# ChuaCheowHuan/gym-continuousDoubleAuction

Hardware: AMD Instinct MI355X
Metric: agent-steps/sec (whole node), 4 agents x N parallel markets; step() with every info tensor (row a14), 4 free-running group chain(s) (higher is better)
Workload: dtype int32+dec28+f64

## Files before the change

gym_continuousdoubleauction_amd/csrc/cda_book.inc:

```
constexpr int CAP = CDA_CAP;
__host__ __device__ constexpr int book_phys(int s, int i) { return s == 0 ? i : CAP - 1 - i; }
struct BookField {
    int32_t v[CAP];
    struct Row { int32_t* base; int s; __device__ __forceinline__ int32_t& operator[](int i) const { return base[book_phys(s, i)]; } };
    struct CRow { const int32_t* base; int s; __device__ __forceinline__ const int32_t& operator[](int i) const { return base[book_phys(s, i)]; } };
    __device__ __forceinline__ Row operator[](int s) { return Row{v, s}; }
    __device__ __forceinline__ CRow operator[](int s) const { return CRow{v, s}; }
};
struct Book {
    BookField price, qty;
    BookField oo;
    BookField ts;
};
constexpr int BOOK_BYTES = sizeof(Book);
enum { TL_N = 0, TL_BASE = 2, TL_PTR_LO = 4, TL_PTR_HI = 5, TL_CAP = 6, TL_ORD = 8, TL_WORDS = 12 };
struct Lds {
    Book book;
    int32_t lvl_px[2][CDA_K_ROWS];
    int32_t lvl_sz[2][CDA_K_ROWS];
    int32_t act_tsp[CDA_MAX_AGENTS];
    int32_t act_size[CDA_MAX_AGENTS];
    int32_t tl[TL_WORDS];
    Acc acc[CDA_MAX_AGENTS];
};
// ... 340 lines not shown
            if (i < tn) { T.field(s, 0)[to] = v0; T.field(s, 1)[to] = v1; T.field(s, 2)[to] = v2; T.field(s, 3)[to] = v3; }
        }
    }
    L.tl[TL_BASE + s] = base; L.tl[TL_N + s] = tn - 1;
    CDA_WSYNC();
    tail_fence();
}
CDA_COLD void cold_aggregate(uint32_t lds_addr, int s, int t, int carry) {
    Lds& L = lds_at(lds_addr);
    const Tail T = tail_of(L);
    const int lane = lane_id();
    const int base = L.tl[TL_BASE + s], tn = L.tl[TL_N + s];
    int32_t prev = t > 0 ? L.book.price[s][t - 1] : -1;
    for (int b = 0; b < tn && carry <= CDA_K_ROWS; b += WAVE) {
        const int i = b + lane;
        const bool valid = i < tn;
        int32_t p = 0, q = 0;
        if (valid) { const uint32_t sl = T.slot(base, i); p = T.field(s, 0)[sl]; q = T.field(s, 1)[sl]; }
        const int32_t up = __shfl(p, (lane + 63) & 63, WAVE);
        const int32_t pp = lane == 0 ? prev : up;
        const bool head = valid && p != pp;
        const uint64_t mk = __ballot(head);
        const uint64_t le = lane == 63 ? ~0ull : ((1ull << (lane + 1)) - 1ull);
        const int lvl = carry + __popcll(mk & le) - 1;
        if (valid && lvl >= 0 && lvl < CDA_K_ROWS) {
            atomicAdd(&L.lvl_sz[s][lvl], q);
            if (head) L.lvl_px[s][lvl] = p;
        }
        carry += __popcll(mk);
        prev = __builtin_amdgcn_readlane(p, 63);
    }
    CDA_WSYNC();
}
__device__ __forceinline__ void sync_tail_status(const Lds& L, Mkt& m) {
    m.status = (m.status & ~ST_TAIL_ANY) | (L.tl[TL_N] > 0 ? ST_TAIL_BID : 0) | (L.tl[TL_N + 1] > 0 ? ST_TAIL_ASK : 0);
}
__device__ __forceinline__ void set_counts(Mkt& m, uint32_t counts) { m.nb = (int32_t)(counts & 0x7fffu); m.na = (int32_t)((counts >> 16) & 0x7fffu); }
__device__ __forceinline__ int total_orders(const Lds& L, const Mkt& m) { return m.nb + m.na + ((m.status & ST_TAIL_ANY) ? L.tl[TL_N] + L.tl[TL_N + 1] : 0); }
#define ACC_UPD(field, expr) do { D _r = (expr); st_dec(a.field, _r, flags); } while (0)
__device__ __forceinline__ void xfer_inc(Acc& a, bool counter, D v, uint32_t& flags) {
    cda_dec& fld = counter ? a.hold : a.cash;
    D r = d_sub(ld_dec(fld), v);
    st_dec(fld, r, flags);
}
__device__ __forceinline__ void xfer_dec(Acc& a, bool counter, D v, uint32_t& flags) {
    ACC_UPD(cash, d_add(ld_dec(a.cash), v));
    if (counter) { ACC_UPD(hold, d_sub(ld_dec(a.hold), v)); ACC_UPD(cash, d_add(ld_dec(a.cash), v)); }
}
__device__ __forceinline__ D posval_from(Acc& a, uint32_t n, int32_t price, bool is_long) {
    D raw = d_mul_int(ld_dec(a.vwap), n), mkt = d_price_times(price, n);
    return d_add(raw, cal_profit(is_long, mkt, raw));
}
template <bool LAZY_POSVAL>
__device__ __forceinline__ void settle_fill(Lds& L, int tr, int counter, int32_t q, int32_t price, int init_side, uint32_t& flags, int lane CDA_TF_PARAM) {
    uint32_t f = 0;
    TF_BEGIN();
    const int al = lane_acc(lane), g = lane_grp(lane);
    if (counter != tr) {
        if ((al == tr || al == counter) && g < 3) {
            Acc& a = L.acc[al];
            const bool is_counter = al == counter;
            const int own_side = is_counter ? init_side ^ 1 : init_side;
            int4 cnt = *reinterpret_cast<const int4*>(&a.net_position);
            const D vwap0 = ld_dec(a.vwap);
            const int32_t pos = cnt.x;
            const uint32_t ap = (uint32_t)(pos < 0 ? -pos : pos);
            const bool is_long = pos > 0;
            int mode;
            if (pos == 0) mode = 0;
            else if (is_long == (own_side == S_BID)) mode = 1;
            else mode = ap > (uint32_t)q ? 2 : (ap == (uint32_t)q ? 3 : 4);
            const D tv = d_price_times(price, (uint32_t)q);
            D X = d_zero(), mkt = d_zero();
            TF_END(14);
            if (g == 0 && mode != 0) X = d_mul_int(vwap0, ap);
            TF_END(15);
            D x2 = d_zero(), y2 = d_zero();
            cda_dec* dst = nullptr;
            bool s2 = false;
            if (g == 0) {
                s2 = true;
                if (mode == 0) { x2 = ld_dec(a.posval); y2 = tv; dst = &a.posval; }
                else if (mode <= 2) { x2 = X; y2 = tv; y2.sign = mode == 2 ? 1 : 0; }
                else { mkt = d_price_times(price, ap); x2 = is_long ? mkt : X; y2 = d_neg(is_long ? X : mkt); }
            } else if (mode <= 2) {
                if (g == 1) {
                    s2 = true;
                    dst = (mode != 2 && is_counter) ? &a.hold : &a.cash;
                    x2 = ld_dec(*dst); y2 = tv; y2.sign = mode != 2 ? 1 : 0;
                } else if (mode == 2 && is_counter) {
                    s2 = true;
                    dst = &a.hold; x2 = ld_dec(a.hold); y2 = d_neg(tv);
                }
            }
            D Y = d_zero();
            TF_END(16);
            if (s2) { Y = d_add(x2, y2); if (dst) st_dec(*dst, Y, f); }
            TF_END(17);
            if (g == 0) {
                cnt.y += 1; cnt.z += 1; cnt.w += is_counter ? 1 : 0;
                if (mode == 0) st_dec(a.vwap, d_price(price), f);
                else if (mode <= 2) {
                    const uint32_t n = mode == 1 ? ap + (uint32_t)q : ap - (uint32_t)q;
                    ACC_UPD(vwap, d_div_u32(Y, n));
                    if (!LAZY_POSVAL) ACC_UPD(posval, posval_from(a, n, price, is_long));
                    if (mode == 2 && is_counter) ACC_UPD(cash, d_add(ld_dec(a.cash), tv));
                } else {
                    D pv = d_add(X, Y);
                    ACC_UPD(cash, d_add(ld_dec(a.cash), d_sub(pv, mkt)));
                    st_dec(a.posval, d_zero(), f); st_dec(a.vwap, d_zero(), f);
                    if (mode == 3) xfer_dec(a, is_counter, tv, f);
                    else {
                        xfer_dec(a, is_counter, mkt, f);
                        D npv = d_price_times(price, (uint32_t)q - ap);
                        st_dec(a.posval, npv, f); st_dec(a.vwap, d_price(price), f);
                        xfer_inc(a, is_counter, npv, f);
                    }
                }
                int64_t np = (int64_t)pos + (own_side == S_BID ? (int64_t)q : -(int64_t)q);
                if (np > 2147483647LL || np < -2147483647LL) f |= CDA_FLAG_INT_OVERFLOW << 8;
                cnt.x = (int32_t)np;
                *reinterpret_cast<int4*>(&a.net_position) = cnt;
            }
            if (mode >= 3) { TF_END(22); TF_COUNT(21); } else if (g == 0 && mode == 0) { TF_END(23); TF_COUNT(12); } else TF_END(18);
            TF_COUNT(20);
        }
        CDA_WSYNC();
        TF_WAVE(tr, counter);
        TF_RESYNC();
    } else if (lane == tr) {
        Acc& a = L.acc[lane];
        D tv = d_price_times(price, (uint32_t)q);
        D hold = d_sub(ld_dec(a.hold), tv), cash = d_add(ld_dec(a.cash), tv);
        st_dec(a.hold, hold, f); st_dec(a.cash, cash, f);
    }
    if (__ballot((f & 0xffu) != 0)) flags |= CDA_FLAG_DEC_DOMAIN;
    if (__ballot((f >> 8) != 0)) flags |= CDA_FLAG_INT_OVERFLOW;
    TF_END(19);
    TF_WAVE_END();
}

template <bool TAILS, bool LAZY_POSVAL>
__device__ __forceinline__ int32_t match(Lds& L, Mkt& m, int tr, int own_side, int32_t qty, int32_t limit, int lane) {
    int opp = own_side ^ 1;
    Book& bk = L.book;
    for (;;) {
        int h = 0;
        const int nopp = mkt_n(m, opp);
        while (qty > 0 && h < nopp) {
            int32_t p = bk.price[opp][h];
            if (limit >= 0) { if (own_side == S_BID ? !(limit >= p) : !(limit <= p)) break; }
            int32_t rq = bk.qty[opp][h], c = oo_owner(bk.oo[opp][h]), f;
            if (qty < rq) { f = qty; bk.qty[opp][h] = rq - qty; qty = 0; CDA_WSYNC(); }
            else { f = rq; qty -= rq; h++; }
            m.has_trade = 1; m.last_trade_price = p;
            TACC_COUNT(m, 5, 1);
            m.fills += 1;
            if (m.fills == 1) __builtin_amdgcn_s_setprio(1);
            else if (m.fills == 2) __builtin_amdgcn_s_setprio(2);
            else if (m.fills == 3) __builtin_amdgcn_s_setprio(3);
            if (!CDA_MKT_DBG(m, 0x1000)) settle_fill<LAZY_POSVAL>(L, tr, c, f, p, own_side, m.flags, lane CDA_TF_ARG(m));
        }
        if (h) { book_remove(bk, opp, nopp, 0, h, lane); mkt_set_n(m, opp, nopp - h); }
        if constexpr (TAILS) {
            if (!mkt_has_tail(m, opp)) break;
            const bool ran_out = qty > 0 && h == nopp;
            set_counts(m, cold_rebalance(lds_addr_of(L), pack_counts(m.nb, m.na)));
            sync_tail_status(L, m);
            if (!ran_out || mkt_n(m, opp) == 0) break;
        } else break;
    }
    return qty;
}

__device__ __forceinline__ void cash_hold_transfer(Lds& L, int tr, int32_t price, int32_t qty, int cash_dir, uint32_t& flags, int lane) {
    const int g = lane_grp(lane);
    if (lane_acc(lane) == tr && g < 2) {
        Acc& a = L.acc[tr];
        D v = d_price_times(price, (uint32_t)qty);
        cda_dec& fld = g == 0 ? a.cash : a.hold;
        v.sign = (g == 0) == (cash_dir > 0) ? 0 : 1;
        const D cur = ld_dec(fld);
        D r = d_add_order_value(cur, v);
        if (r.exp == D_NOT_HANDLED) r = d_add(cur, v);
        st_dec(fld, r, flags);
    }
    CDA_WSYNC();
}

__device__ __forceinline__ bool order_approved(Lds& L, const Mkt& m, int tr, int side, int32_t size, int32_t price, int lane) {
    int ok = 0;
    if (lane == tr) {
        const Acc& a = L.acc[lane];
        const D nav = ld_dec(a.nav), cash = ld_dec(a.cash);
        const int32_t pos32 = a.net_position;
        const int32_t opp_best = L.book.price[side ^ 1][0];
        if (d_sgn(nav) > 0) {
            int64_t pos = pos32, opening;
            int64_t apos = pos < 0 ? -pos : pos;
            if ((side == S_BID && pos >= 0) || (side == S_ASK && pos <= 0)) opening = size;
            else { opening = (int64_t)size - apos; if (opening < 0) opening = 0; }
            if (opening <= 0) ok = 1;
            else {
                D est;
                if (price < 0) {
                    int opp = side ^ 1;
                    if (mkt_n(m, opp) > 0) est = d_price(opp_best);
                    else if (m.has_trade) est = d_price(m.last_trade_price);
                    else est = d_from_u32(1);
                } else est = d_price(price);
                uint64_t ov = (uint64_t)((uint32_t)est.w0) * (uint64_t)opening;
                int kdig = est.exp - cash.exp;
                int bc = bits128(d_c128(cash)), bo = 64 - __clzll(ov | 1ull);
                if (!cash.sign && kdig >= 0 && kdig <= 30 && opening < (1LL << 31) && bc - 1 >= bo + ((kdig * 3402) >> 10) + 1) ok = 1;
                else ok = d_cmp(cash, d_mul_u32(est, (uint32_t)opening, 0)) >= 0;
            }
        }
    }
    return __ballot(ok != 0) != 0;
}

template <bool TAILS, bool LAZY_POSVAL>
__device__ __forceinline__ void place_order(Lds& L, Mkt& m, int tr, int type, int side, int32_t size, int32_t price, int lane) {
    if (side == S_NONE) return;
// ... 189 lines not shown
```

gym_continuousdoubleauction_amd/csrc/cda_dec.hpp:

```cpp
#pragma once
#include <hip/hip_runtime.h>
#include <stdint.h>

typedef unsigned __int128 u128;

namespace cda {

#ifdef CDA_DEC_COUNTERS
__device__ unsigned long long g_dec_calls[8];
#define DEC_COUNT(i) atomicAdd(&g_dec_calls[i], 1ull)
#else
#define DEC_COUNT(i) do {} while (0)
#endif

template <int NL> struct WN { uint32_t w[NL]; };
typedef WN<8> W;
typedef WN<4> W4;

struct D {
    uint32_t w0, w1, w2;
    int32_t exp;
    int32_t sign;
};

// ... 187 lines not shown
__device__ __forceinline__ D d_from_i64(int64_t v) {
    uint64_t a = v < 0 ? (uint64_t)(-(v + 1)) + 1u : (uint64_t)v;
    return d_make((uint32_t)a, (uint32_t)(a >> 32), 0, 0, v < 0);
}
__device__ __forceinline__ D d_from_u32(uint32_t v) { return d_make(v, 0, 0, 0, 0); }
__device__ __forceinline__ D d_price(int32_t p) { uint64_t a = (uint64_t)(uint32_t)p * 10u; return d_make((uint32_t)a, (uint32_t)(a >> 32), 0, -1, 0); }
__device__ __forceinline__ D d_price_times(int32_t p, uint32_t n) {
    const uint64_t c = (uint64_t)(uint32_t)p * 10u * (uint64_t)n;
    return d_make((uint32_t)c, (uint32_t)(c >> 32), 0, -1, 0);
}
__device__ __forceinline__ bool d_is_zero(const D& a) { return (a.w0 | a.w1 | a.w2) == 0; }
template <int NL> __device__ __forceinline__ WN<NL> d_wide(const D& a) { return w_from3<NL>(a.w0, a.w1, a.w2); }
__device__ __forceinline__ D d_neg(D a) { a.sign ^= 1; return a; }
__device__ __forceinline__ int d_sgn(const D& a) { return d_is_zero(a) ? 0 : (a.sign ? -1 : 1); }

template <int NL> __device__ __forceinline__ D d_fix_impl(int sign, WN<NL> x, int exp) {
    if (w_is_zero(x)) return d_make(0, 0, 0, exp, sign);
    int nd = w_ndigits(x);
    if (nd > 28) {
        int drop = nd - 28;
        bool sticky = false;
        int k = drop;
        while (k > 9) { sticky |= (w_divc<1000000000u>(x) != 0); k -= 9; }
        uint32_t rem = w_div_pow10_small(x, k);
        uint32_t half = 5u * pow10_sel(k - 1);
        bool up = rem > half || (rem == half && (sticky || (x.w[0] & 1u)));
        if (up) {
            w_inc(x);
            if (x.w[0] == 0x10000000u && x.w[1] == 0x3e250261u && x.w[2] == 0x204fce5eu) {
                x.w[0] = 0xe8000000u; x.w[1] = 0x9fd0803cu; x.w[2] = 0x033b2e3cu; drop += 1;
            }
        }
        exp += drop;
    }
    return d_make(x.w[0], x.w[1], x.w[2], exp, sign);
}
__device__ __noinline__ D d_fix_mid(int sign, W4 x, int exp) { DEC_COUNT(0); return d_fix_impl<4>(sign, x, exp); }
__device__ __noinline__ D d_fix_wide(int sign, W x, int exp) { DEC_COUNT(1); return d_fix_impl<8>(sign, x, exp); }

__device__ __forceinline__ u128 d_c128(const D& a) { return ((u128)a.w2 << 64) | ((u128)a.w1 << 32) | (u128)a.w0; }
__device__ __forceinline__ D d_from128(u128 c, int exp, int sign) { return d_make((uint32_t)c, (uint32_t)(c >> 32), (uint32_t)(c >> 64), exp, sign); }
__device__ __forceinline__ W4 w4_from128(u128 c) { W4 r; r.w[0] = (uint32_t)c; r.w[1] = (uint32_t)(c >> 32); r.w[2] = (uint32_t)(c >> 64); r.w[3] = (uint32_t)(c >> 96); return r; }
__device__ __forceinline__ u128 p28_128() { return ((u128)0x204fce5eULL << 64) | 0x3e25026110000000ULL; }
__device__ __forceinline__ int bits128(u128 c) {
    uint64_t hi = (uint64_t)(c >> 64), lo = (uint64_t)c;
    return hi ? 128 - __clzll(hi) : (lo ? 64 - __clzll(lo) : 0);
}
__device__ __forceinline__ u128 mul_pow10_128(u128 x, int k) {
    while (k >= 9) { x *= (u128)1000000000u; k -= 9; }
    return x * (u128)pow10_sel(k);
}
__device__ __forceinline__ bool scale_fits128(u128 c, int k) { return bits128(c) + ((k * 3402) >> 10) + 1 <= 126; }

__device__ __noinline__ D d_round_mid(int sign, u128 r, int exp) {
    DEC_COUNT(2);
    const int t = (bits128(r) * 1233) >> 12;
    const int d0 = t - 28, d0c = d0 > 9 ? 9 : d0, d1c = d0 + 1 > 9 ? 9 : d0 + 1;
    const lds_u32p pt = lds_pow10(t);
    const uint32_t t0 = pt[0], t1 = pt[1], t2 = pt[2], t3 = pt[3];
    const uint32_t pw_a = lds_pow10(d0c)[0], pw_b = lds_pow10(d1c)[0];
    const double rd_a = lds_rcp10(d0c), rd_b = lds_rcp10(d1c);
    const u128 pw_t = ((u128)t3 << 96) | ((u128)t2 << 64) | ((u128)t1 << 32) | (u128)t0;
    const bool more = r >= pw_t;
    int drop = d0 + (more ? 1 : 0);
    exp += drop;
    W4 x = w4_from128(r);
    bool sticky = false;
    uint32_t pw = more ? pw_b : pw_a;
    double rd = more ? rd_b : rd_a;
    if (drop > 9) {
        const int pre = drop - 9;
        sticky = w_div_small(x, lds_pow10(pre)[0], lds_rcp10(pre)) != 0;
        drop = 9; pw = 1000000000u; rd = lds_rcp10(9);
    }
    WN<3> q; q.w[0] = x.w[0]; q.w[1] = x.w[1]; q.w[2] = x.w[2];
    const uint32_t rem = w_div_small_seeded(q, pw, rd, x.w[3]);
    const uint32_t half = pw >> 1;
    const bool up = rem > half || (rem == half && (sticky || (q.w[0] & 1u) != 0));
    const uint64_t s0 = (uint64_t)q.w[0] + (up ? 1u : 0u);
    const uint64_t s1 = (uint64_t)q.w[1] + (s0 >> 32);
    uint32_t w0 = (uint32_t)s0, w1 = (uint32_t)s1, w2 = q.w[2] + (uint32_t)(s1 >> 32);
    const bool ten28 = w0 == 0x10000000u && w1 == 0x3e250261u && w2 == 0x204fce5eu;
    w0 = ten28 ? 0xe8000000u : w0; w1 = ten28 ? 0x9fd0803cu : w1; w2 = ten28 ? 0x033b2e3cu : w2;
    exp += ten28 ? 1 : 0;
    return d_make(w0, w1, w2, exp, sign);
}

__device__ __noinline__ D d_add_wide(D a, D b) {
    DEC_COUNT(3);
    int exp = a.exp < b.exp ? a.exp : b.exp;
    bool az = d_is_zero(a), bz = d_is_zero(b);
    if (az && bz) return d_make(0, 0, 0, exp, a.sign < b.sign ? a.sign : b.sign);
    if (az || bz) {
        D o = az ? b : a;
        int e = exp > o.exp - 29 ? exp : o.exp - 29;
        W x = d_wide<8>(o);
        w_mul_pow10(x, o.exp - e);
        return d_fix_wide(o.sign, x, e);
    }
    bool swp = a.exp < b.exp;
    D dt = swp ? b : a, dO = swp ? a : b;
    W xt = d_wide<8>(dt), xo = d_wide<8>(dO);
    int et = dt.exp, eo = dO.exp;
    if (et != eo) {
        int tmp_len = w_ndigits(xt), oth_len = w_ndigits(xo);
        int m = tmp_len - 30; if (m > -1) m = -1;
        int e = et + m;
        if (oth_len + eo - 1 < e) { xo = w_from3<8>(1, 0, 0); eo = e; }
        w_mul_pow10(xt, et - eo);
    }
    W r; int rs;
    if (dt.sign != dO.sign) {
        int c = w_cmp(xt, xo);
        if (c == 0) return d_make(0, 0, 0, exp, 0);
        if (c > 0) { r = w_sub(xt, xo); rs = dt.sign; } else { r = w_sub(xo, xt); rs = dO.sign; }
    } else { r = w_add(xt, xo); rs = dt.sign; }
    return d_fix_wide(rs, r, eo);
}
__device__ __noinline__ D d_add_mid(D a, D b) {
    DEC_COUNT(4);
    bool swp = a.exp < b.exp;
    D t = swp ? b : a, o = swp ? a : b;
    int diff = t.exp - o.exp;
    u128 ct = d_c128(t), co = d_c128(o);
    bool ok = true;
    if (diff) {
        int lb_adj = o.exp + (((bits128(co) - 1) * 1233) >> 12);
        ok = scale_fits128(ct, diff) && lb_adj >= t.exp - 1;
    }
    if (!ok) return d_add_wide(a, b);
    if (diff) ct = mul_pow10_128(ct, diff);
    u128 r; int rs;
    if (t.sign != o.sign) {
        if (ct == co) return d_make(0, 0, 0, o.exp, 0);
        if (ct > co) { r = ct - co; rs = t.sign; } else { r = co - ct; rs = o.sign; }
    } else { r = ct + co; rs = t.sign; }
    if (r < p28_128()) return d_from128(r, o.exp, rs);
    return d_round_mid(rs, r, o.exp);
}
__device__ __forceinline__ u128 mul_u32_pow10_lds(uint32_t c, int k) {
    const lds_u32p p = lds_pow10(k);
    u128 pw = ((u128)p[2] << 64) | ((u128)p[1] << 32) | (u128)p[0];
    return pw * (u128)c;
}
__device__ __forceinline__ D d_add(D a, D b) {
    const bool az = d_is_zero(a), bz = d_is_zero(b);
    if (!az && !bz) {
        const bool swp = a.exp < b.exp;
        const D t = swp ? b : a, o = swp ? a : b;
        const int diff = t.exp - o.exp;
        const u128 co = d_c128(o);
        u128 ct;
        bool ok;
        if (diff == 0) { ct = d_c128(t); ok = true; }
        else {
            ok = (((bits128(co) - 1) * 1233) >> 12) >= diff - 1;
            if ((t.w1 | t.w2) == 0 && diff <= 28) ct = mul_u32_pow10_lds(t.w0, diff);
            else if (diff <= 9) ct = d_c128(t) * (u128)lds_pow10(diff)[0];
            else { ok = false; ct = 0; }
        }
        if (ok) {
            u128 r; int rs;
            if (t.sign != o.sign) {
                if (ct == co) return d_make(0, 0, 0, o.exp, 0);
                if (ct > co) { r = ct - co; rs = t.sign; } else { r = co - ct; rs = o.sign; }
            } else { r = ct + co; rs = t.sign; }
            if (r < p28_128()) return d_from128(r, o.exp, rs);
            return d_round_mid(rs, r, o.exp);
        }
        return d_add_mid(a, b);
    }
    if (az != bz) {
        const D o = az ? b : a, z = az ? a : b;
        if (z.exp >= o.exp) return o;
    }
    return d_add_wide(a, b);
}
__device__ __forceinline__ D d_sub(D a, D b) { return d_add(a, d_neg(b)); }
constexpr int D_NOT_HANDLED = -0x40000000;
__device__ __noinline__ D d_add_order_value(D field, D v) {
    const int diff = v.exp - field.exp;
    const u128 co = d_c128(field);
    const bool fz = co == 0;
    const int dcl = diff < 0 ? 0 : (diff > 28 ? 28 : diff);
    const bool shape = (v.w1 | v.w2) == 0 && v.w0 != 0 && diff == dcl &&
                       (fz || (((bits128(co) - 1) * 1233) >> 12) >= diff - 1);
    const u128 ct = mul_u32_pow10_lds(v.w0, dcl);
    const bool same = field.sign == v.sign || fz;
    const bool vg = ct > co;
    const u128 sum = ct + co, dv = ct - co, df = co - ct;
    const u128 r = same ? sum : (vg ? dv : df);
    int rs = same ? (fz ? v.sign : field.sign) : (vg ? v.sign : field.sign);
    rs = r == 0 ? 0 : rs;
    const bool ok = shape && r < p28_128();
    return d_make(ok ? (uint32_t)r : 0u, ok ? (uint32_t)(r >> 32) : 0u, ok ? (uint32_t)(r >> 64) : 0u, ok ? field.exp : D_NOT_HANDLED, ok ? rs : 0);
}

__device__ __forceinline__ D d_mul_u32(D a, uint32_t m, int mexp) {
    int exp = a.exp + mexp;
    if (d_is_zero(a) || m == 0) return d_make(0, 0, 0, exp, a.sign);
    u128 p = d_c128(a) * (u128)m;
    if (p < p28_128()) return d_from128(p, exp, a.sign);
    return d_round_mid(a.sign, p, exp);
}
__device__ __forceinline__ D d_mul_int(D a, uint32_t n) { return d_mul_u32(a, n, 0); }

template <int NL> __device__ __forceinline__ uint32_t w_mod5(const WN<NL>& x) {
    uint64_t sacc = 0;
    #pragma unroll
    for (int i = 0; i < NL; i++) sacc += x.w[i];
    return (uint32_t)(sacc % 5u);
}
template <int NL> __device__ __forceinline__ D d_div_impl(D a, uint32_t n, int shift) {
    WN<NL> x = d_wide<NL>(a);
    int exp = a.exp - shift;
    w_mul_pow10(x, shift);
    uint32_t rem = w_div_u32(x, n);
    if (rem != 0) {
        if (w_mod5(x) == 0) w_inc(x);
        WN<NL> p29 = w_pow10<NL>(29);
        const bool d30 = w_cmp(x, p29) >= 0;
        uint32_t dg, half;
        if (d30) { dg = w_divc<100u>(x); half = 50u; exp += 2; } else { dg = w_divc<10u>(x); half = 5u; exp += 1; }
        if (dg > half || (dg == half && (x.w[0] & 1u))) {
            w_inc(x);
            if (x.w[0] == 0x10000000u && x.w[1] == 0x3e250261u && x.w[2] == 0x204fce5eu) {
                x.w[0] = 0xe8000000u; x.w[1] = 0x9fd0803cu; x.w[2] = 0x033b2e3cu; exp += 1;
            }
        }
        return d_make(x.w[0], x.w[1], x.w[2], exp, a.sign);
    }
    int ideal = a.exp;
    while (exp + 9 <= ideal) { WN<NL> t = x; if (w_divc<1000000000u>(t) != 0) break; x = t; exp += 9; }
    while (exp < ideal) { WN<NL> t = x; if (w_divc<10u>(t) != 0) break; x = t; exp += 1; }
    return d_fix_impl<NL>(a.sign, x, exp);
}
__device__ __noinline__ D d_div_general(D a, uint32_t n) {
    DEC_COUNT(5);
    if (d_is_zero(a)) return d_make(0, 0, 0, a.exp, a.sign);
    {
        WN<3> x; x.w[0] = a.w0; x.w[1] = a.w1; x.w[2] = a.w2;
        if (w_div_u32(x, n) == 0) return d_make(x.w[0], x.w[1], x.w[2], a.exp, a.sign);
    }
    W4 xa = d_wide<4>(a), xn = w_from3<4>(n, 0, 0);
    int ln = w_ndigits(xn);
    int shift = ln - w_ndigits(xa) + 29;
    if (ln <= 9) return d_div_impl<4>(a, n, shift);
    return d_div_impl<8>(a, n, shift);
}
__device__ __forceinline__ int ndigits_u32(uint32_t n) {
    int d = 1;
    d = n >= 10u ? 2 : d; d = n >= 100u ? 3 : d; d = n >= 1000u ? 4 : d; d = n >= 10000u ? 5 : d; d = n >= 100000u ? 6 : d;
    d = n >= 1000000u ? 7 : d; d = n >= 10000000u ? 8 : d; d = n >= 100000000u ? 9 : d; d = n >= 1000000000u ? 10 : d;
    return d;
}
__device__ __noinline__ D d_div_pos_leaf(D a, uint32_t n) {
    DEC_COUNT(6);
    if (n - 1u >= (1u << 30) - 1u) return d_make(0, 0, 0, D_NOT_HANDLED, 0);
    const double rn = 1.0 / (double)n;
    const u128 c = d_c128(a);
    WN<3> q; q.w[0] = a.w0; q.w[1] = a.w1; q.w[2] = a.w2;
    int s = 0;
    if (w_div_small(q, n, rn) != 0) {
        const int t = (bits128(c) * 1233) >> 12;
        const lds_u32p pt = lds_pow10(t);
        const u128 pw_t = ((u128)pt[2] << 64) | ((u128)pt[1] << 32) | (u128)pt[0];
        const int s0 = 27 + ndigits_u32(n) - (t + (c >= pw_t ? 1 : 0));
        const lds_u32p ps = lds_pow10(s0);
        const u128 pw_s = ((u128)ps[3] << 96) | ((u128)ps[2] << 64) | ((u128)ps[1] << 32) | (u128)ps[0];
        const u128 x0 = c * pw_s;
        const u128 n27 = (u128)n * (((u128)0x033b2e3cULL << 64) | 0x9fd0803ce8000000ULL);
        const bool d28 = x0 >= n27;
        s = s0 + (d28 ? 0 : 1);
        W4 x = w4_from128(d28 ? x0 : x0 * 10u);
        const uint32_t r = w_div_small(x, n, rn);
        q.w[0] = x.w[0]; q.w[1] = x.w[1]; q.w[2] = x.w[2];
        if (r != 0) {
            const uint32_t twice = r * 2u;
            const bool up = twice > n || (twice == n && (q.w[0] & 1u) != 0);
            const uint64_t s0w = (uint64_t)q.w[0] + (up ? 1u : 0u);
            const uint64_t s1w = (uint64_t)q.w[1] + (s0w >> 32);
            uint32_t w0 = (uint32_t)s0w, w1 = (uint32_t)s1w, w2 = q.w[2] + (uint32_t)(s1w >> 32);
            const bool ten28 = w0 == 0x10000000u && w1 == 0x3e250261u && w2 == 0x204fce5eu;
            w0 = ten28 ? 0xe8000000u : w0; w1 = ten28 ? 0x9fd0803cu : w1; w2 = ten28 ? 0x033b2e3cu : w2;
            return d_make(w0, w1, w2, a.exp - s + (ten28 ? 1 : 0), a.sign);
        }
        #pragma unroll 1
        while (s >= 4) { WN<3> u = q; if (w_divc<10000u>(u) != 0) break; q = u; s -= 4; }
        #pragma unroll 1
        while (s >= 1) { WN<3> u = q; if (w_divc<10u>(u) != 0) break; q = u; s -= 1; }
    }
    return d_make(q.w[0], q.w[1], q.w[2], a.exp - s, a.sign);
}
__device__ __forceinline__ D d_div_u32(D a, uint32_t n) {
    D r = d_div_pos_leaf(a, n);
    if (r.exp == D_NOT_HANDLED) r = d_div_general(a, n);
    return r;
}

__device__ __noinline__ int d_cmp_wide(D a, D b) {
    int s = a.sign ? -1 : 1;
    int diff = a.exp - b.exp;
    if (diff >= 28) return s;
    if (diff <= -28) return -s;
    W xa = d_wide<8>(a), xb = d_wide<8>(b);
    if (diff > 0) w_mul_pow10(xa, diff); else if (diff < 0) w_mul_pow10(xb, -diff);
    int c = w_cmp(xa, xb);
    return c == 0 ? 0 : (c > 0 ? s : -s);
}
__device__ __noinline__ int d_cmp_mid(D a, D b) {
    int s = a.sign ? -1 : 1;
    int diff = a.exp - b.exp;
    u128 ca = d_c128(a), cb = d_c128(b);
    if (diff > 0) { if (!scale_fits128(ca, diff)) return d_cmp_wide(a, b); ca = mul_pow10_128(ca, diff); }
    else if (diff < 0) { if (!scale_fits128(cb, -diff)) return d_cmp_wide(a, b); cb = mul_pow10_128(cb, -diff); }
    return ca == cb ? 0 : (ca > cb ? s : -s);
}
__device__ __forceinline__ int d_cmp(D a, D b) {
    const bool az = d_is_zero(a), bz = d_is_zero(b);
    if (az) return bz ? 0 : (b.sign ? 1 : -1);
    if (bz) return a.sign ? -1 : 1;
    if (a.sign != b.sign) return a.sign ? -1 : 1;
    const int s = a.sign ? -1 : 1;
    const bool swp = a.exp < b.exp;
    const D t = swp ? b : a, o = swp ? a : b;
    const int diff = t.exp - o.exp;
    const bool short_t = (t.w1 | t.w2) == 0;
    if (!(short_t ? diff <= 28 : diff <= 9)) return d_cmp_mid(a, b);
    const lds_u32p p = lds_pow10(diff);
    const uint32_t p0 = p[0], p1 = p[1], p2 = p[2];
    const u128 big = short_t ? (((u128)p2 << 64) | ((u128)p1 << 32) | (u128)p0) : d_c128(t);
    const u128 ct = big * (u128)(short_t ? t.w0 : p0), co = d_c128(o);
    const int c = ct == co ? 0 : (ct > co ? s : -s);
    return swp ? -c : c;
}

__device__ __forceinline__ double round_quotient(uint64_t q, bool sticky, int t, int k) {
    int nb = 64 - __clzll(q);
    int sh = nb - 53;
    uint64_t mant = q >> sh;
    uint64_t low = q & (((uint64_t)1 << sh) - 1);
    uint64_t half = (uint64_t)1 << (sh - 1);
    if (low > half || (low == half && (sticky || (mant & 1)))) mant += 1;
    return ldexp((double)mant, t - 56 + sh - k);
}
__device__ __forceinline__ void w_shl(W& x, int n) {
    int ws = n >> 5, bs = n & 31;
    W r;
// ... 142 lines not shown
```

gym_continuousdoubleauction_amd/csrc/cda_hip.hip:

```cpp
#include <hip/hip_runtime.h>
#include <stdint.h>
#include <stdio.h>
#include <stdlib.h>
#include <string.h>
#include <math.h>
#include <dlfcn.h>

#include "../../include/cda.h"
#include "../../include/cda_random_agents.h"
#include "cda_dec.hpp"
#include "cda_market.hpp"
#include <type_traits>
#include <mutex>
#include "../../include/cda_mlp.h"
namespace cda { namespace mlpdev {
#include "cda_mlp_dev.inc"
} }
#undef CDA_MLP_HIST
#define CDA_MLP_HIST 1
namespace cda { namespace mlpdev_h1 {
#include "cda_mlp_dev.inc"
} }
#undef CDA_MLP_HIST
#define CDA_MLP_HIST 2
// ... 424 lines not shown
        cda_random_action(seed, market_base + (uint64_t)mk, (uint32_t)(step0 + (int)t), (uint32_t)a, &category[ix], &size_mean[ix], &size_sigma[ix], &price[ix], &price_offset[ix]);
    }
}
__global__ __launch_bounds__(256) void k_handback_unpack(const uint8_t* rec, int n_seg, int seg_records, long long seg_row_stride, long long row0, int A, int H, int stride,
                                                          long long n_rows_total, float* obs_full, double* reward_full, uint8_t* term_full, uint8_t* trunc_full) {
    const long long r = (long long)(((size_t)blockIdx.x * blockDim.x + threadIdx.x) >> 6);
    const int lane = (int)(threadIdx.x & 63);
    if (r >= (long long)n_seg * seg_records) return;
    const uint8_t* p = rec + (size_t)r * (size_t)stride;
    const long long seg = r / seg_records, local = row0 + (r % seg_records);
    if (n_rows_total > 0 && local >= (seg == n_seg - 1 ? n_rows_total - seg * seg_row_stride : seg_row_stride)) return;
    const size_t row = (size_t)(seg * seg_row_stride + local);
    const uint8_t* fl = p + CDA_SNAPSHOT_DIM * 4 + A * 8;
    const bool restarted = fl[2] != 0;
    if (lane < CDA_SNAPSHOT_DIM) {
        float* o = obs_full + row * (size_t)(H * CDA_SNAPSHOT_DIM);
        const float nf = reinterpret_cast<const float*>(p)[lane];
        float keep[CDA_MAX_HIST];
        #pragma unroll
        for (int h = 1; h < CDA_MAX_HIST; h++) keep[h] = h < H ? o[h * CDA_SNAPSHOT_DIM + lane] : 0.0f;
        #pragma unroll
        for (int h = 1; h < CDA_MAX_HIST; h++) if (h < H) o[(h - 1) * CDA_SNAPSHOT_DIM + lane] = restarted ? nf : keep[h];
        o[(H - 1) * CDA_SNAPSHOT_DIM + lane] = nf;
    }
    if (lane < A) reward_full[row * (size_t)A + (size_t)lane] = reinterpret_cast<const double*>(p + CDA_SNAPSHOT_DIM * 4)[lane];
    if (lane == 0) { term_full[row] = fl[0]; trunc_full[row] = fl[1]; }
}
__global__ void k_book_peak(const uint8_t* arena, Params P, int32_t* out) {
    int i = (int)(blockIdx.x * blockDim.x + threadIdx.x);
    if (i < P.n_markets) out[i] = (int32_t)((const uint32_t*)(arena + (size_t)i * (size_t)P.lay.stride))[H_PEAK_ORDERS];
}

__global__ void k_selftest_dec(int op, int n, const cda_dec* a, const cda_dec* b, cda_dec* out) {
    int i = (int)(blockIdx.x * blockDim.x + threadIdx.x);
    dec_tables_init();
    if (i >= n) return;
    D x = ld_dec(a[i]);
    D y = b ? ld_dec(b[i]) : d_zero();
    cda_dec o; o.w[0] = o.w[1] = o.w[2] = 0; o.exp = 0; o.sign = 0; o.pad = 0;
    uint32_t f = 0;
    uint32_t yc = y.w0;
    switch (op) {
        case 0: st_dec(o, d_add(x, y), f); break;
        case 1: st_dec(o, d_sub(x, y), f); break;
        case 2: { D r = d_mul_u32(x, yc, y.exp); r.sign ^= y.sign; st_dec(o, r, f); break; }
        case 3: { D r = d_div_u32(x, yc); r.sign ^= y.sign; st_dec(o, r, f); break; }
        case 4: o.w[0] = (uint32_t)(d_cmp(x, y) + 1); break;
        case 6: {
            D r = d_add_order_value(x, y);
            const bool handled = r.exp != D_NOT_HANDLED;
            if (!handled) r = d_add(x, y);
            st_dec(o, r, f); o.pad = handled ? 1u : 0u; break;
        }
        default: { double d = d_to_double(x, &f); unsigned long long bits = (unsigned long long)__double_as_longlong(d); o.w[0] = (uint32_t)bits; o.w[1] = (uint32_t)(bits >> 32); o.w[2] = f; break; }
    }
    out[i] = o;
}
__global__ void k_selftest_libm(int op, int n, const double* x, double* y) {
    int i = (int)(blockIdx.x * blockDim.x + threadIdx.x);
    if (i < n) y[i] = op == 0 ? glibc_log1p(x[i]) : (op == 1 ? glibc_exp(x[i]) : sqrt(x[i]));
}
__global__ void k_selftest_rng(uint64_t seed, int lo, int hi, int n_steps, int n_normals, int perm_n,
                               int32_t* first_int, double* normals, int32_t* perms, uint64_t* final_state) {
    if (threadIdx.x != 0 || blockIdx.x != 0) return;
    Mkt m; rng_seed(m, seed);
    *first_int = rng_integers(m, lo, hi);
    for (int s = 0; s < n_steps; s++) {
        for (int k = 0; k < n_normals; k++) normals[(size_t)s * (size_t)n_normals + (size_t)k] = rng_std_normal(m);
        int32_t* p = perms + (size_t)s * (size_t)perm_n;
        for (int i = 0; i < perm_n; i++) p[i] = i;
        for (int i = perm_n - 1; i >= 1; i--) { int j = (int)rng_interval(m, (uint32_t)i); int32_t t = p[i]; p[i] = p[j]; p[j] = t; }
    }
    final_state[0] = (uint64_t)(m.rng_state >> 64); final_state[1] = (uint64_t)m.rng_state;
    final_state[2] = (uint64_t)(m.rng_inc >> 64); final_state[3] = (uint64_t)m.rng_inc;
    final_state[4] = m.has_u32; final_state[5] = m.uinteger;
}

struct cda_env {
    Params P;
    int device;
    int cap;
    uint8_t* arena;
    size_t arena_bytes;
    uint8_t* done_buf;
    uint8_t* handback;
    int64_t hb_row_stride, hb_rows_total;
    int32_t spill_wanted;
    double* em_partials;
    MktRow* rows;
    cda_market_params* rows_host;
    uint32_t* snap_flag;
};
static inline int32_t handback_stride_of(int32_t num_agents) { return (CDA_SNAPSHOT_DIM * 4 + num_agents * 8 + 3 + 7) & ~7; }

static thread_local char g_err[256] = "";
static int g_dbg_skip = 0;
static unsigned long long* g_phase_cycles = NULL;
static int hip_fail(hipError_t e, const char* what) {
    snprintf(g_err, sizeof g_err, "%s: %s", what, hipGetErrorString(e));
    return CDA_ERR_HIP;
}
#define HIPCHK(x) do { hipError_t _e = (x); if (_e != hipSuccess) return hip_fail(_e, #x); } while (0)

extern "C" {

const char* cda_strerror(int status) {
// ... 745 lines not shown
        }
        h[H_PEAK_ORDERS] = (uint32_t)(s->n_bids + s->n_asks);
    }
    h[H_RNG_STATE_LO] = (uint32_t)s->rng_state_lo; h[H_RNG_STATE_LO + 1] = (uint32_t)(s->rng_state_lo >> 32);
    h[H_RNG_STATE_HI] = (uint32_t)s->rng_state_hi; h[H_RNG_STATE_HI + 1] = (uint32_t)(s->rng_state_hi >> 32);
    h[H_RNG_INC_LO] = (uint32_t)s->rng_inc_lo; h[H_RNG_INC_LO + 1] = (uint32_t)(s->rng_inc_lo >> 32);
    h[H_RNG_INC_HI] = (uint32_t)s->rng_inc_hi; h[H_RNG_INC_HI + 1] = (uint32_t)(s->rng_inc_hi >> 32);
    h[H_HAS_U32] = s->rng_has_uint32; h[H_UINTEGER] = s->rng_uinteger;
    h[H_T_STEP] = (uint32_t)s->t_step; h[H_LOB_TIME] = (uint32_t)s->lob_time; h[H_NEXT_OID] = (uint32_t)s->next_order_id;
    h[H_LAST_PRICE] = (uint32_t)s->last_price; h[H_HAS_TRADE] = (uint32_t)s->has_trade; h[H_LAST_TRADE_PRICE] = (uint32_t)s->last_trade_price;
    h[H_DONE_MASK] = s->done_mask; h[H_FLAGS] = s->flags;
    h[H_SEEDED] = 1; h[H_HIST_HEAD] = 0;
    Acc* ap = (Acc*)(rec + P.lay.acc_off);
    for (int a = 0; a < P.cfg.num_agents; a++) {
        const cda_account_state* o = &s->acc[a];
        ap[a].cash = o->cash; ap[a].hold = o->cash_on_hold; ap[a].posval = o->position_val; ap[a].vwap = o->vwap;
        ap[a].nav = o->nav; ap[a].prev_nav = o->prev_nav; ap[a].max_nav = o->max_nav;
        ap[a].net_position = o->net_position; ap[a].num_trades = o->num_trades;
        ap[a].num_trades_step = o->num_trades_step; ap[a].num_passive_fills_step = o->num_passive_fills_step;
        ap[a].order_step_placed = o->order_step_placed; ap[a].num_rejected_step = o->num_rejected_step;
    }
    memcpy(rec + P.lay.hist_off, s->hist, sizeof(float) * (size_t)P.cfg.n_hist * CDA_SNAPSHOT_DIM);
    hipError_t he = hipMemcpy(rec + P.lay.ep_off, dev_rec + P.lay.ep_off, (size_t)P.cfg.num_agents * sizeof(EpStats), hipMemcpyDeviceToHost);
    if (he == hipSuccess) he = hipMemcpy(dev_rec, rec, (size_t)P.lay.stride, hipMemcpyHostToDevice);
    free(rec);
    if (he != hipSuccess) return hip_fail(he, "hipMemcpy H2D");
    return CDA_OK;
}

int cda_get_raw_snapshot(cda_env* e, float* raw_out, void* stream) {
    if (!e || !raw_out) return CDA_ERR_INVALID;
    HIPCHK(hipSetDevice(e->device));
    LAUNCH_CAP(e, k_raw_snapshot, grid_for(e->P.n_markets), dim3(64 * CDA_WPB), smem_for(e, CDA_WPB), (hipStream_t)stream, e->arena, e->P, raw_out);
    HIPCHK(hipGetLastError());
    return CDA_OK;
}
int cda_last_flags(cda_env* e, uint32_t* flags_out, void* stream) {
    if (!e || !flags_out) return CDA_ERR_INVALID;
    HIPCHK(hipSetDevice(e->device));
    hipLaunchKernelGGL(k_flags, dim3((unsigned)((e->P.n_markets + 255) / 256)), dim3(256), 0, (hipStream_t)stream, e->arena, e->P, flags_out);
    HIPCHK(hipGetLastError());
    return CDA_OK;
}

int cda_check_invariants(cda_env* e, uint32_t* violations_out, void* stream) {
    if (!e || !violations_out) return CDA_ERR_INVALID;
    HIPCHK(hipSetDevice(e->device));
    hipLaunchKernelGGL(k_check_invariants, dim3((unsigned)((e->P.n_markets + 63) / 64)), dim3(64), 0, (hipStream_t)stream, (const uint8_t*)e->arena, e->P, e->cap, violations_out);
    HIPCHK(hipGetLastError());
    return CDA_OK;
}

int cda_selftest_dec(int32_t device, int32_t op, int32_t n, const cda_dec* a_host, const cda_dec* b_host, cda_dec* out_host) {
    if (n < 0 || !a_host || !out_host || op < 0 || op > 6) return CDA_ERR_INVALID;
    int ndev = 0;
    if (hipGetDeviceCount(&ndev) != hipSuccess || ndev <= 0) return CDA_ERR_NO_DEVICE;
    HIPCHK(hipSetDevice(device));
    if (n == 0) return CDA_OK;
    cda_dec *da = NULL, *db = NULL, *dout = NULL;
    size_t bytes = (size_t)n * sizeof(cda_dec);
    HIPCHK(hipMalloc((void**)&da, bytes)); HIPCHK(hipMalloc((void**)&dout, bytes));
    HIPCHK(hipMemcpy(da, a_host, bytes, hipMemcpyHostToDevice));
    if (b_host) { HIPCHK(hipMalloc((void**)&db, bytes)); HIPCHK(hipMemcpy(db, b_host, bytes, hipMemcpyHostToDevice)); }
    hipLaunchKernelGGL(k_selftest_dec, dim3((unsigned)((n + 63) / 64)), dim3(64), DEC_TABLE_BYTES, 0, op, n, da, db, dout);
    HIPCHK(hipGetLastError());
    HIPCHK(hipDeviceSynchronize());
    HIPCHK(hipMemcpy(out_host, dout, bytes, hipMemcpyDeviceToHost));
    (void)hipFree(da); (void)hipFree(dout); if (db) (void)hipFree(db);
    return CDA_OK;
}

int cda_selftest_libm(int32_t device, int32_t op, int32_t n, const double* x_host, double* y_host) {
    if (n < 0 || !x_host || !y_host || op < 0 || op > 2) return CDA_ERR_INVALID;
    int ndev = 0;
    if (hipGetDeviceCount(&ndev) != hipSuccess || ndev <= 0) return CDA_ERR_NO_DEVICE;
    HIPCHK(hipSetDevice(device));
    if (n == 0) return CDA_OK;
    double *dx = NULL, *dy = NULL;
    const size_t bytes = (size_t)n * sizeof(double);
    HIPCHK(hipMalloc((void**)&dx, bytes)); HIPCHK(hipMalloc((void**)&dy, bytes));
    HIPCHK(hipMemcpy(dx, x_host, bytes, hipMemcpyHostToDevice));
    hipLaunchKernelGGL(k_selftest_libm, dim3((unsigned)((n + 255) / 256)), dim3(256), 0, 0, (int)op, (int)n, dx, dy);
    HIPCHK(hipGetLastError());
    HIPCHK(hipDeviceSynchronize());
    HIPCHK(hipMemcpy(y_host, dy, bytes, hipMemcpyDeviceToHost));
    (void)hipFree(dx); (void)hipFree(dy);
    return CDA_OK;
}
int cda_selftest_libm_host(int32_t op, int32_t n, const double* x_host, double* y_host) {
    if (n < 0 || !x_host || !y_host || op < 0 || op > 1) return CDA_ERR_INVALID;
    for (int32_t i = 0; i < n; i++) y_host[i] = op == 0 ? glibc_log1p(x_host[i]) : glibc_exp(x_host[i]);
    return CDA_OK;
}

int cda_selftest_rng(int32_t device, uint64_t seed, int32_t lo, int32_t hi, int32_t n_steps, int32_t n_normals, int32_t perm_n,
                     int32_t* first_int_host, double* normals_host, int32_t* perms_host, uint64_t* final_state_host) {
    if (n_steps < 0 || n_normals < 0 || perm_n < 0 || !first_int_host || !final_state_host) return CDA_ERR_INVALID;
    int ndev = 0;
    if (hipGetDeviceCount(&ndev) != hipSuccess || ndev <= 0) return CDA_ERR_NO_DEVICE;
    HIPCHK(hipSetDevice(device));
    int32_t* dfi = NULL; double* dn = NULL; int32_t* dp = NULL; uint64_t* dfs = NULL;
    size_t nb = sizeof(double) * (size_t)n_steps * (size_t)n_normals + 8, pb = sizeof(int32_t) * (size_t)n_steps * (size_t)perm_n + 8;
    HIPCHK(hipMalloc((void**)&dfi, 8)); HIPCHK(hipMalloc((void**)&dn, nb)); HIPCHK(hipMalloc((void**)&dp, pb)); HIPCHK(hipMalloc((void**)&dfs, 64));
    hipLaunchKernelGGL(k_selftest_rng, dim3(1), dim3(64), 0, 0, seed, lo, hi, n_steps, n_normals, perm_n, dfi, dn, dp, dfs);
    HIPCHK(hipGetLastError());
    HIPCHK(hipDeviceSynchronize());
    HIPCHK(hipMemcpy(first_int_host, dfi, 4, hipMemcpyDeviceToHost));
// ... 33 lines not shown
```

Measured before the change: 458.0 million.

## Inline decimal rounding/division in fill settlement and defer flag ballots to match end

Adds FILL template variants of d_add, d_mul_u32 and d_div_u32 that inline the rounding and division leaf bodies instead of calling noinline functions. settle_fill uses them in its hot arithmetic. It also accumulates error flags into a per-lane word across the whole match loop and does the two wave ballots once at the end instead of per fill. The aim is to cut call overhead and per-fill cross-lane ballots, at the cost of larger code and higher register pressure in the fill path. New selftest ops 7-9 exercise the inlined variants.

Measured after the change: 461.4 million (median of 6 runs). No clear change (+0.7%).

```diff
diff --git a/gym_continuousdoubleauction_amd/csrc/cda_book.inc b/gym_continuousdoubleauction_amd/csrc/cda_book.inc
--- a/gym_continuousdoubleauction_amd/csrc/cda_book.inc
+++ b/gym_continuousdoubleauction_amd/csrc/cda_book.inc
@@ -416,8 +416,7 @@
     return d_add(raw, cal_profit(is_long, mkt, raw));
 }
 template <bool LAZY_POSVAL>
-__device__ __forceinline__ void settle_fill(Lds& L, int tr, int counter, int32_t q, int32_t price, int init_side, uint32_t& flags, int lane CDA_TF_PARAM) {
-    uint32_t f = 0;
+__device__ __forceinline__ void settle_fill(Lds& L, int tr, int counter, int32_t q, int32_t price, int init_side, uint32_t& flags, uint32_t& f, int lane CDA_TF_PARAM) {
     TF_BEGIN();
     const int al = lane_acc(lane), g = lane_grp(lane);
     if (counter != tr) {
@@ -437,7 +436,7 @@
             const D tv = d_price_times(price, (uint32_t)q);
             D X = d_zero(), mkt = d_zero();
             TF_END(14);
-            if (g == 0 && mode != 0) X = d_mul_int(vwap0, ap);
+            if (g == 0 && mode != 0) X = d_mul_int<true>(vwap0, ap);
             TF_END(15);
             D x2 = d_zero(), y2 = d_zero();
             cda_dec* dst = nullptr;
@@ -459,14 +458,14 @@
             }
             D Y = d_zero();
             TF_END(16);
-            if (s2) { Y = d_add(x2, y2); if (dst) st_dec(*dst, Y, f); }
+            if (s2) { Y = d_add<true>(x2, y2); if (dst) st_dec(*dst, Y, f); }
             TF_END(17);
             if (g == 0) {
                 cnt.y += 1; cnt.z += 1; cnt.w += is_counter ? 1 : 0;
                 if (mode == 0) st_dec(a.vwap, d_price(price), f);
                 else if (mode <= 2) {
                     const uint32_t n = mode == 1 ? ap + (uint32_t)q : ap - (uint32_t)q;
-                    ACC_UPD(vwap, d_div_u32(Y, n));
+                    ACC_UPD(vwap, d_div_u32<true>(Y, n));
                     if (!LAZY_POSVAL) ACC_UPD(posval, posval_from(a, n, price, is_long));
                     if (mode == 2 && is_counter) ACC_UPD(cash, d_add(ld_dec(a.cash), tv));
                 } else {
@@ -498,8 +497,6 @@
         D hold = d_sub(ld_dec(a.hold), tv), cash = d_add(ld_dec(a.cash), tv);
         st_dec(a.hold, hold, f); st_dec(a.cash, cash, f);
     }
-    if (__ballot((f & 0xffu) != 0)) flags |= CDA_FLAG_DEC_DOMAIN;
-    if (__ballot((f >> 8) != 0)) flags |= CDA_FLAG_INT_OVERFLOW;
     TF_END(19);
     TF_WAVE_END();
 }
@@ -508,6 +505,7 @@
 __device__ __forceinline__ int32_t match(Lds& L, Mkt& m, int tr, int own_side, int32_t qty, int32_t limit, int lane) {
     int opp = own_side ^ 1;
     Book& bk = L.book;
+    uint32_t ff = 0;
     for (;;) {
         int h = 0;
         const int nopp = mkt_n(m, opp);
@@ -523,7 +521,7 @@
             if (m.fills == 1) __builtin_amdgcn_s_setprio(1);
             else if (m.fills == 2) __builtin_amdgcn_s_setprio(2);
             else if (m.fills == 3) __builtin_amdgcn_s_setprio(3);
-            if (!CDA_MKT_DBG(m, 0x1000)) settle_fill<LAZY_POSVAL>(L, tr, c, f, p, own_side, m.flags, lane CDA_TF_ARG(m));
+            if (!CDA_MKT_DBG(m, 0x1000)) settle_fill<LAZY_POSVAL>(L, tr, c, f, p, own_side, m.flags, ff, lane CDA_TF_ARG(m));
         }
         if (h) { book_remove(bk, opp, nopp, 0, h, lane); mkt_set_n(m, opp, nopp - h); }
         if constexpr (TAILS) {
@@ -534,6 +532,8 @@
             if (!ran_out || mkt_n(m, opp) == 0) break;
         } else break;
     }
+    if (__ballot((ff & 0xffu) != 0)) m.flags |= CDA_FLAG_DEC_DOMAIN;
+    if (__ballot((ff >> 8) != 0)) m.flags |= CDA_FLAG_INT_OVERFLOW;
     return qty;
 }
 
diff --git a/gym_continuousdoubleauction_amd/csrc/cda_dec.hpp b/gym_continuousdoubleauction_amd/csrc/cda_dec.hpp
--- a/gym_continuousdoubleauction_amd/csrc/cda_dec.hpp
+++ b/gym_continuousdoubleauction_amd/csrc/cda_dec.hpp
@@ -263,8 +263,7 @@
 }
 __device__ __forceinline__ bool scale_fits128(u128 c, int k) { return bits128(c) + ((k * 3402) >> 10) + 1 <= 126; }
 
-__device__ __noinline__ D d_round_mid(int sign, u128 r, int exp) {
-    DEC_COUNT(2);
+__device__ __forceinline__ D d_round_mid_impl(int sign, u128 r, int exp) {
     const int t = (bits128(r) * 1233) >> 12;
     const int d0 = t - 28, d0c = d0 > 9 ? 9 : d0, d1c = d0 + 1 > 9 ? 9 : d0 + 1;
     const lds_u32p pt = lds_pow10(t);
@@ -296,6 +295,7 @@
     exp += ten28 ? 1 : 0;
     return d_make(w0, w1, w2, exp, sign);
 }
+__device__ __noinline__ D d_round_mid(int sign, u128 r, int exp) { DEC_COUNT(2); return d_round_mid_impl(sign, r, exp); }
 
 __device__ __noinline__ D d_add_wide(D a, D b) {
     DEC_COUNT(3);
@@ -354,6 +354,7 @@
     u128 pw = ((u128)p[2] << 64) | ((u128)p[1] << 32) | (u128)p[0];
     return pw * (u128)c;
 }
+template <bool FILL = false>
 __device__ __forceinline__ D d_add(D a, D b) {
     const bool az = d_is_zero(a), bz = d_is_zero(b);
     if (!az && !bz) {
@@ -377,7 +378,7 @@
                 if (ct > co) { r = ct - co; rs = t.sign; } else { r = co - ct; rs = o.sign; }
             } else { r = ct + co; rs = t.sign; }
             if (r < p28_128()) return d_from128(r, o.exp, rs);
-            return d_round_mid(rs, r, o.exp);
+            return FILL ? d_round_mid_impl(rs, r, o.exp) : d_round_mid(rs, r, o.exp);
         }
         return d_add_mid(a, b);
     }
@@ -387,7 +388,8 @@
     }
     return d_add_wide(a, b);
 }
-__device__ __forceinline__ D d_sub(D a, D b) { return d_add(a, d_neg(b)); }
+template <bool FILL = false>
+__device__ __forceinline__ D d_sub(D a, D b) { return d_add<FILL>(a, d_neg(b)); }
 constexpr int D_NOT_HANDLED = -0x40000000;
 __device__ __noinline__ D d_add_order_value(D field, D v) {
     const int diff = v.exp - field.exp;
@@ -407,14 +409,16 @@
     return d_make(ok ? (uint32_t)r : 0u, ok ? (uint32_t)(r >> 32) : 0u, ok ? (uint32_t)(r >> 64) : 0u, ok ? field.exp : D_NOT_HANDLED, ok ? rs : 0);
 }
 
+template <bool FILL = false>
 __device__ __forceinline__ D d_mul_u32(D a, uint32_t m, int mexp) {
     int exp = a.exp + mexp;
     if (d_is_zero(a) || m == 0) return d_make(0, 0, 0, exp, a.sign);
     u128 p = d_c128(a) * (u128)m;
     if (p < p28_128()) return d_from128(p, exp, a.sign);
-    return d_round_mid(a.sign, p, exp);
-}
-__device__ __forceinline__ D d_mul_int(D a, uint32_t n) { return d_mul_u32(a, n, 0); }
+    return FILL ? d_round_mid_impl(a.sign, p, exp) : d_round_mid(a.sign, p, exp);
+}
+template <bool FILL = false>
+__device__ __forceinline__ D d_mul_int(D a, uint32_t n) { return d_mul_u32<FILL>(a, n, 0); }
 
 template <int NL> __device__ __forceinline__ uint32_t w_mod5(const WN<NL>& x) {
     uint64_t sacc = 0;
@@ -465,8 +469,7 @@
     d = n >= 1000000u ? 7 : d; d = n >= 10000000u ? 8 : d; d = n >= 100000000u ? 9 : d; d = n >= 1000000000u ? 10 : d;
     return d;
 }
-__device__ __noinline__ D d_div_pos_leaf(D a, uint32_t n) {
-    DEC_COUNT(6);
+__device__ __forceinline__ D d_div_pos_impl(D a, uint32_t n) {
     if (n - 1u >= (1u << 30) - 1u) return d_make(0, 0, 0, D_NOT_HANDLED, 0);
     const double rn = 1.0 / (double)n;
     const u128 c = d_c128(a);
@@ -503,8 +506,10 @@
     }
     return d_make(q.w[0], q.w[1], q.w[2], a.exp - s, a.sign);
 }
+__device__ __noinline__ D d_div_pos_leaf(D a, uint32_t n) { DEC_COUNT(6); return d_div_pos_impl(a, n); }
+template <bool FILL = false>
 __device__ __forceinline__ D d_div_u32(D a, uint32_t n) {
-    D r = d_div_pos_leaf(a, n);
+    D r = FILL ? d_div_pos_impl(a, n) : d_div_pos_leaf(a, n);
     if (r.exp == D_NOT_HANDLED) r = d_div_general(a, n);
     return r;
 }
diff --git a/gym_continuousdoubleauction_amd/csrc/cda_hip.hip b/gym_continuousdoubleauction_amd/csrc/cda_hip.hip
--- a/gym_continuousdoubleauction_amd/csrc/cda_hip.hip
+++ b/gym_continuousdoubleauction_amd/csrc/cda_hip.hip
@@ -500,6 +500,9 @@
             if (!handled) r = d_add(x, y);
             st_dec(o, r, f); o.pad = handled ? 1u : 0u; break;
         }
+        case 7: { D r = d_mul_u32<true>(x, yc, y.exp); r.sign ^= y.sign; st_dec(o, r, f); break; }
+        case 8: st_dec(o, d_add<true>(x, y), f); break;
+        case 9: { D r = d_div_u32<true>(x, yc); r.sign ^= y.sign; st_dec(o, r, f); break; }
         default: { double d = d_to_double(x, &f); unsigned long long bits = (unsigned long long)__double_as_longlong(d); o.w[0] = (uint32_t)bits; o.w[1] = (uint32_t)(bits >> 32); o.w[2] = f; break; }
     }
     out[i] = o;
@@ -1351,7 +1354,7 @@
 }
 
 int cda_selftest_dec(int32_t device, int32_t op, int32_t n, const cda_dec* a_host, const cda_dec* b_host, cda_dec* out_host) {
-    if (n < 0 || !a_host || !out_host || op < 0 || op > 6) return CDA_ERR_INVALID;
+    if (n < 0 || !a_host || !out_host || op < 0 || op > 9) return CDA_ERR_INVALID;
     int ndev = 0;
     if (hipGetDeviceCount(&ndev) != hipSuccess || ndev <= 0) return CDA_ERR_NO_DEVICE;
     HIPCHK(hipSetDevice(device));
```
